# merthidayetoglu/HiCCL

Measured on AMD Instinct MI355X. Metric: GB/s device-resident N-way float bucket sum, 1 GB/input; % HBM peak, higher is better.
Workload: dtype f32

## Files before the change

### hiccl_amd/csrc/oneshot.cpp

```cpp
#include <string.h>

#include "plan.h"

using namespace hiccl_impl;

namespace {

uint32_t log2u(int v) {
  uint32_t l = 0;
  while (v > 1) {
    v >>= 1;
    l++;
  }
  return l;
}

int reduce_via_table(int dtype, const Cfg &c, void *out, const void *const *in, int n, size_t count,
                     hipStream_t s) {
  DescTable t((size_t)n, unit_pkts(c.engine, dtype, c.acc, c.unroll));
  t.add(out, in, (size_t)n, count, esize(dtype));
  const std::vector<char> host = t.image();
  char *dmem = nullptr;
  if (int e = check_hip(hipMallocAsync((void **)&dmem, host.size(), s), "hiccl_reduce: hipMallocAsync")) return e;
  if (int e = check_hip(hipMemcpyAsync(dmem, host.data(), host.size(), hipMemcpyHostToDevice, s),
                        "hiccl_reduce: table upload")) {
    (void)hipFreeAsync(dmem, s);
    return e;
  }
  PlanArgs a;
  memset(&a, 0, sizeof(a));
  t.bind(a, dmem);
  a.t_begin = 0;
  a.t_end = t.units;
  const int pol = plan_pol(c.store == kPolStoreSys ? HICCL_PEER_STORES : 0);
  if (int e = launch_plan(a, dtype, c, n, current_device(), s, pol)) {
    (void)hipFreeAsync(dmem, s);
    return e;
  }
  return check_hip(hipFreeAsync(dmem, s), "hiccl_reduce: hipFreeAsync");
}

}

extern "C" {

int hiccl_reduce_ex(int dtype, void *out, const void *const *in, int n, size_t count,
                    void *stream, const hiccl_reduce_config_t *cfg) {
  const size_t esz = esize(dtype);
  if (!esz) return fail(hipErrorInvalidValue, "hiccl_reduce: unknown dtype " + std::to_string(dtype));
  if (count == 0) return 0;
  if (dtype == HICCL_BYTES && n != 1) return fail(hipErrorInvalidValue, "hiccl_reduce: HICCL_BYTES copies need n == 1");
  if (int e = check_buffers(out, in, n, count, esz)) return e;
  if (int e = check_cfg(cfg, "hiccl_reduce")) return e;
  hipStream_t s = (hipStream_t)stream;
  const int dev = current_device();
  Split sp = split_on(out, count, esz);
  Cfg c = oneshot_cfg(dtype, cfg, sp.npkt, (uint64_t)count * esz, n, dev);
  if (n > kMaxArgInputs) {
    const std::string why = plan_shape_error(c, dtype);
    if (!why.empty()) return fail(hipErrorInvalidValue, "hiccl_reduce_ex: n > 64 inputs run on the plan kernel: " + why);
    if (capturing(s, false))
      return fail(hipErrorStreamCaptureUnsupported,
                  "hiccl_reduce: n > 64 inputs cannot be captured into a graph (use a plan)");
    return reduce_via_table(dtype, c, out, in, n, count, s);
  }

  single_fn fn = single_for(dtype, c);
  if (!fn)
    return fail(hipErrorInvalidValue, "hiccl_reduce_ex: unsupported config (block " +
                                          std::to_string(c.block) + ", unroll " +
                                          std::to_string(c.unroll) + ", nt " +
                                          std::to_string(c.nt) + ", store " +
                                          std::to_string(c.store) + ", engine " +
                                          std::to_string(c.engine) + ") for this dtype");

  SingleArgs a;
  memset(&a, 0, sizeof(a));
  a.out = (char *)out;
  a.npkt = sp.npkt;
  a.head = sp.head;
  a.tail = sp.tail;
  a.n = (uint32_t)n;
  a.ntiles = tiles_for(sp.npkt, (uint64_t)c.block * c.unroll);
  for (int k = 0; k < n; k++) a.in[k] = (const char *)in[k];

  const LaunchShape L = launch_shape(c, n, a.ntiles, device_cus(dev));
  a.grab = L.grab;
  a.drain = (uint32_t)c.drain;
  a.order = log2u(c.order);
  a.sched = L.dynamic ? ticket_counter(dev, s) : nullptr;
  fn(a, dim3((unsigned)L.grid), s);
  return check_hip(hipGetLastError(), "hiccl_reduce: launch");
}

int hiccl_reduce(int dtype, void *out, const void *const *in, int n, size_t count, void *stream) {
  return hiccl_reduce_ex(dtype, out, in, n, count, stream, nullptr);
}

int hiccl_reduce_f32(float *out, const float *const *in, int n, size_t count, void *stream) {
  return hiccl_reduce_ex(HICCL_FLOAT32, out, (const void *const *)in, n, count, stream, nullptr);
}

int hiccl_reduce_bf16(uint16_t *out, const uint16_t *const *in, int n, size_t count,
                      void *stream) {
  return hiccl_reduce_ex(HICCL_BFLOAT16, out, (const void *const *)in, n, count, stream, nullptr);
}

int hiccl_reduce_auto_choice_ex(int dtype, const hiccl_reduce_config_t *cfg, size_t count, double n, int cus,
                                int *engine, int *unroll, int *blocks_per_cu, int *dynamic, int *store_policy) {
  const size_t esz = esize(dtype);
  if (!esz) return fail(hipErrorInvalidValue, "auto_choice: unknown dtype");
  if (cus <= 0 || n < 0) return fail(hipErrorInvalidValue, "auto_choice: cus must be > 0 and n >= 0");
  if (int e = check_cfg(cfg, "auto_choice")) return e;
  CusOverride scoped(cus);
  const uint64_t npkt = (uint64_t)count * esz / kPacket;
  const Cfg c = oneshot_cfg(dtype, cfg, npkt, (uint64_t)count * esz, n, -1);
  const bool has = n > kMaxArgInputs ? plan_shape_error(c, dtype).empty() : single_for(dtype, c) != nullptr;
  if (!has) return fail(hipErrorInvalidValue, "auto_choice: no kernel for this config and dtype");
  const uint64_t units = tiles_for(npkt, (uint64_t)c.block * c.unroll);
  const LaunchShape L = launch_shape(c, n, units, cus);
  if (engine) *engine = c.engine;
  if (unroll) *unroll = c.unroll;
  if (blocks_per_cu) *blocks_per_cu = c.bpc;
  if (dynamic) *dynamic = L.dynamic ? 1 : 0;
  if (store_policy) *store_policy = c.store + 1;
  return 0;
}

int hiccl_reduce_auto_choice(int dtype, int acc, size_t count, double n, int cus, int *engine, int *unroll,
                             int *blocks_per_cu, int *dynamic) {
  hiccl_reduce_config_t z;
  memset(&z, 0, sizeof(z));
  z.acc = acc;
  return hiccl_reduce_auto_choice_ex(dtype, &z, count, n, cus, engine, unroll, blocks_per_cu, dynamic, nullptr);
}

}
```

### hiccl_amd/csrc/policy.cpp

```cpp
#include "policy.h"

namespace hiccl_impl {

namespace {

constexpr uint64_t kDynMinUnitsPerWG = 32;
constexpr double kDynMinInputs = 5;
constexpr double kTicketTiles = 9;
constexpr uint64_t kTileMinTicketsPerWG = 64;

constexpr int kWideUnroll = 8;
constexpr uint64_t kWideMinTicketsPerWG = 128;

constexpr uint64_t kWtMaxBytes = 32ull << 20;
constexpr uint64_t kWtMaxBytesReduce = 256ull << 20;
inline uint64_t wt_cap(double n) { return n >= 1.5 ? kWtMaxBytesReduce : kWtMaxBytes; }

constexpr int kDefBpc = 1;
constexpr int kSmallBpc = 4;
constexpr uint64_t kPhaseMinChunksPerCU = 1;

uint32_t default_grab(int engine, double n, int unroll = kDefUnroll) {
  if (engine == HICCL_ENGINE_PHASE || unroll >= kWideUnroll) return 1u;
  const double g = kTicketTiles / (n + 1.0);
  return g <= 1.0 ? 1u : (uint32_t)(g + 0.999);
}

int auto_wide_unroll(uint64_t npkt, double n, int dtype, const Cfg &c, int dev) {
  if (!tuned_type(dtype, c.acc) || n < 1.5 || n >= kDynMinInputs) return 0;
  if ((c.block && c.block != kDefBlock) || c.nt != kDefPol % 10 || c.store != kDefPol / 10) return 0;
  if (npkt / ((uint64_t)kDefBlock * kWideUnroll) < kWideMinTicketsPerWG * (uint64_t)device_cus(dev)) return 0;
  return n < 2.5 ? 2 * kWideUnroll : kWideUnroll;
}

int auto_engine(uint64_t npkt, double n, int dtype, const Cfg &c, int dev) {
  const int acc = c.acc;
  if (auto_wide_unroll(npkt, n, dtype, c, dev)) return HICCL_ENGINE_TILE;
  const bool packed_ok = !(dtype == HICCL_BFLOAT16 && acc == HICCL_ACC_WIDE);
  const bool wt = c.wt;
  const bool wt_f32 = wt && dtype == HICCL_FLOAT32;
  const bool wt_many = wt && tuned_type(dtype, acc);
  if (n >= kDynMinInputs && packed_ok && !wt_many) {
    const uint64_t tickets = npkt / ((uint64_t)kDefBlock * kDefUnroll) / default_grab(HICCL_ENGINE_TILE, n);
    if (tickets >= kTileMinTicketsPerWG * (uint64_t)device_cus(dev)) return HICCL_ENGINE_TILE;
  }
  const uint64_t chunk = (uint64_t)kPhBlock * phase_p(dtype, acc);
  const uint64_t cus = (uint64_t)device_cus(dev);
  const uint64_t per_cu = npkt / (cus * chunk);
  const bool big_chunk = chunk >= 8192;
  const uint64_t chunks = (npkt + chunk - 1) / chunk;
  const double round_eff = chunks ? (double)chunks / (double)(((chunks + cus - 1) / cus) * cus) : 0.0;
  if (n < 2.5) return per_cu > 16 && round_eff >= 0.89 ? HICCL_ENGINE_PHASE : HICCL_ENGINE_TILE;
  if (n >= 2.5 && n < 3.5 && wt_f32) return HICCL_ENGINE_TILE;
  if (n < kDynMinInputs) return per_cu >= 4 && round_eff >= 0.89 ? HICCL_ENGINE_PHASE : HICCL_ENGINE_TILE;
  const bool enough = per_cu >= 1 || (n >= 16 && big_chunk);
  return enough && round_eff >= (big_chunk ? 0.7 : 0.8) ? HICCL_ENGINE_PHASE : HICCL_ENGINE_TILE;
}

int auto_bpc(int engine, uint64_t npkt, int dtype, int acc, int dev) {
  const uint64_t chunk = (uint64_t)kPhBlock * phase_p(dtype, acc);
  return engine == HICCL_ENGINE_TILE && npkt < kPhaseMinChunksPerCU * (uint64_t)device_cus(dev) * chunk
             ? kSmallBpc
             : kDefBpc;
}

int auto_unroll(uint64_t npkt, int dtype, int acc, int dev) {
  return tuned_type(dtype, acc) && npkt < 2ull * device_cus(dev) * kDefBlock * kDefUnroll ? 2 : kDefUnroll;
}

}

Cfg resolve(const hiccl_reduce_config_t *c) {
  Cfg r{0, 0, 0, kDefPol % 10, HICCL_ACC_NATIVE, 0, kDefPol / 10, HICCL_ENGINE_AUTO, HICCL_SCHED_AUTO, 0, 0, true,
        false, 0};
  if (c) {
    r.block = c->block;
    r.unroll = c->unroll;
    if (c->blocks_per_cu) r.bpc = c->blocks_per_cu;
    if (c->nontemporal) r.nt = c->nontemporal - 1;
    r.acc = c->acc;
    r.grid = c->grid;
    if (c->store_policy) r.store = c->store_policy - 1;
    r.store_auto = c->store_policy == 0;
    r.engine = c->engine;
    r.schedule = c->schedule;
    r.grab = c->grab;
    r.drain = c->drain;
    r.order = c->order;
  }
  return r;
}

int check_cfg(const hiccl_reduce_config_t *c, const std::string &who) {
  if (!c) return 0;
  if (c->acc != HICCL_ACC_NATIVE && c->acc != HICCL_ACC_WIDE) return fail(hipErrorInvalidValue, who + ": bad acc mode");
  if (c->engine < HICCL_ENGINE_AUTO || c->engine > HICCL_ENGINE_PHASE)
    return fail(hipErrorInvalidValue, who + ": bad engine");
  if (c->schedule < HICCL_SCHED_AUTO || c->schedule > HICCL_SCHED_DYNAMIC)
    return fail(hipErrorInvalidValue, who + ": bad schedule");
  if (c->grab < 0 || c->grab > 4096) return fail(hipErrorInvalidValue, who + ": bad grab");
  if (c->order < 0 || c->order > 4096 || (c->order & (c->order - 1)))
    return fail(hipErrorInvalidValue, who + ": order must be 0 or a power of two <= 4096");
  if (c->blocks_per_cu < 0 || c->blocks_per_cu > 64) return fail(hipErrorInvalidValue, who + ": blocks_per_cu");
  if (c->grid < 0) return fail(hipErrorInvalidValue, who + ": grid < 0");
  return 0;
}

bool wt_by_size(const Cfg &raw, int dtype, double n, uint64_t out_bytes) {
  const bool u_ok = !raw.unroll || wt_unroll(raw.unroll) || raw.engine == HICCL_ENGINE_PHASE;
  return raw.store_auto && raw.nt == kDefPol % 10 && u_ok && out_bytes <= wt_cap(dtype == HICCL_BYTES ? 1.0 : n);
}

void finish_cfg(Cfg &c, uint64_t npkt, double n, int dtype, int dev) {
  if (c.engine == HICCL_ENGINE_AUTO)
    c.engine = (c.block || c.unroll) ? HICCL_ENGINE_TILE : auto_engine(npkt, n, dtype, c, dev);
  if (c.engine == HICCL_ENGINE_PHASE) {
    if (!c.block) c.block = kPhBlock;
    if (!c.unroll) c.unroll = phase_p(dtype, c.acc);
  } else {
    if (!c.block) c.block = kDefBlock;
    if (!c.unroll) {
      const int wide = auto_wide_unroll(npkt, n, dtype, c, dev);
      c.unroll = wide ? wide : auto_unroll(npkt, dtype, c.acc, dev);
    }
  }
  if (!c.bpc) c.bpc = auto_bpc(c.engine, npkt, dtype, c.acc, dev);
}

Cfg oneshot_cfg(int dtype, const hiccl_reduce_config_t *cfg, uint64_t npkt, uint64_t out_bytes, double n,
                int dev) {
  const Cfg raw = resolve(cfg);
  Cfg c = raw;
  c.wt = wt_by_size(raw, dtype, n, out_bytes);
  finish_cfg(c, npkt, n, dtype, dev);
  if (!c.wt) return c;
  Cfg w = c;
  w.store = kPolStoreSys;
  if (n > kMaxArgInputs ? pick_plan(dtype, w.acc, w.engine, w.unroll, plan_pol(HICCL_PEER_STORES)) != nullptr
                        : single_for(dtype, w) != nullptr)
    return w;
  c = raw;
  finish_cfg(c, npkt, n, dtype, dev);
  return c;
}

int plan_pol(int peer) {
  return 10 * ((peer & HICCL_PEER_STORES) ? kPolStoreSys : kDefPol / 10) +
         ((peer & HICCL_PEER_LOADS) ? kPolLoadSys : kDefPol % 10);
}

uint64_t unit_pkts(int engine, int dtype, int acc, int unroll) {
  return engine == HICCL_ENGINE_PHASE ? (uint64_t)kPhBlock * phase_p(dtype, acc)
                                      : (uint64_t)kDefBlock * (unroll ? unroll : kDefUnroll);
}

std::string plan_shape_error(const Cfg &c, int dtype) {
  if (c.nt != kDefPol % 10 || (c.store != kDefPol / 10 && c.store != kPolStoreSys))
    return "plan kernels load nt (nontemporal 2) and store nt (store_policy 2), system-scope write-through "
           "(store_policy 4) or either by the launch's size (store_policy 0)";
  if (c.drain) return "plan kernels do not support drain";
  if (c.order != 0 && c.order != 1) return "plan kernels run their units in linear order (order 0)";
  if (c.engine == HICCL_ENGINE_PHASE) {
    if (c.block != kPhBlock || c.unroll != phase_p(dtype, c.acc))
      return "plan kernels run the PHASE engine in its default shape only (block 512, unroll " +
             std::to_string(phase_p(dtype, c.acc)) + ")";
    return "";
  }
  if (c.block != kDefBlock) return "plan kernels run the TILE engine at block 256 only";
  const bool wt = c.store == kPolStoreSys;
  if (wt && !wt_unroll(c.unroll))
    return "write-through plan kernels (store_policy 4) run the TILE engine at unroll 4 (f32 / bf16: 2 or 4) only";
  if (!pick_plan(dtype, c.acc, HICCL_ENGINE_TILE, c.unroll, plan_pol(wt ? HICCL_PEER_STORES : 0)))
    return "plan kernels run the TILE engine at unroll 4 (f32 / bf16: 1, 2, 4, 8 or 16) only";
  return "";
}

LaunchShape launch_shape(const Cfg &c, double n, uint64_t units, int cus) {
  LaunchShape L;
  L.grid = c.grid > 0 ? (uint64_t)c.grid : (uint64_t)cus * c.bpc;
  if (L.grid > units) L.grid = units;
  L.grab = c.grab > 0 ? (uint32_t)c.grab : default_grab(c.engine, n, c.unroll);
  const bool auto_static = c.engine != HICCL_ENGINE_TILE || (n < kDynMinInputs && c.unroll < kWideUnroll);
  L.dynamic = c.schedule != HICCL_SCHED_STATIC && !(c.schedule == HICCL_SCHED_AUTO && auto_static) &&
              (units + L.grab - 1) / L.grab >= kDynMinUnitsPerWG * L.grid;
  return L;
}

}
```

### hiccl_amd/csrc/policy.h

```cpp
#pragma once

#include <string>

#include "runtime.h"

namespace hiccl_impl __attribute__((visibility("hidden"))) {

struct Cfg {
  int block, unroll, bpc, nt, acc, grid, store, engine, schedule, grab, drain;
  bool store_auto;
  bool wt;
  int order;
  int pol() const { return store * 10 + nt; }
};

Cfg resolve(const hiccl_reduce_config_t *c);

int check_cfg(const hiccl_reduce_config_t *c, const std::string &who);

bool wt_by_size(const Cfg &raw, int dtype, double n, uint64_t out_bytes);
inline bool wt_unroll(int unroll) { return unroll == 2 || unroll == kDefUnroll; }

void finish_cfg(Cfg &c, uint64_t npkt, double n, int dtype, int dev);

Cfg oneshot_cfg(int dtype, const hiccl_reduce_config_t *cfg, uint64_t npkt, uint64_t out_bytes, double n, int dev);
inline single_fn single_for(int dtype, const Cfg &c) {
  return pick_single(dtype, c.acc, c.engine, c.block, c.unroll, c.pol());
}

int plan_pol(int peer);
uint64_t unit_pkts(int engine, int dtype, int acc, int unroll);
std::string plan_shape_error(const Cfg &c, int dtype);

struct LaunchShape {
  uint64_t grid;
  uint32_t grab;
  bool dynamic;
};
LaunchShape launch_shape(const Cfg &c, double n, uint64_t units, int cus);

}
```

### hiccl_amd/csrc/reduce.hip

```cpp

#include <hip/hip_runtime.h>

#include <stdint.h>

#include <type_traits>

#include "../../include/hiccl_reduce.h"
#include "kernels.h"

using namespace hiccl_impl;

namespace {


typedef uint32_t u32x4 __attribute__((ext_vector_type(4)));
typedef uint32_t u32x4u __attribute__((ext_vector_type(4), aligned(1)));
typedef float f32x4 __attribute__((ext_vector_type(4)));
typedef double f64x2 __attribute__((ext_vector_type(2)));
typedef uint64_t u64x2 __attribute__((ext_vector_type(2)));
typedef float f32x8 __attribute__((ext_vector_type(8)));
typedef __bf16 bf16x2 __attribute__((ext_vector_type(2)));

typedef __amdgpu_buffer_rsrc_t rsrc_t;
constexpr int kRsrcFlags = 0x00020000;

__device__ __forceinline__ rsrc_t make_rsrc(const char *base, uint32_t nbytes) {
  return __builtin_amdgcn_make_buffer_rsrc((void *)base, (short)0, (int)nbytes, kRsrcFlags);
}

template <int POL>
__device__ __forceinline__ u32x4 load_pkt(rsrc_t r, uint32_t voff) {
  constexpr int lp = POL % 10;
  return __builtin_amdgcn_raw_buffer_load_b128(r, (int)voff, 0, lp == 1 ? 2 : lp == kPolLoadSys ? 17 : 0);
}

template <int POL>
__device__ __forceinline__ void store_pkt(rsrc_t r, uint32_t voff, u32x4 v) {
  constexpr int sp = POL / 10;
  __builtin_amdgcn_raw_buffer_store_b128(v, r, (int)voff, 0, sp == 1 ? 2 : sp == 2 ? 16 : sp == kPolStoreSys ? 17 : 0);
}

__device__ __forceinline__ float bf_lo(uint32_t w) { return __uint_as_float(w << 16); }
__device__ __forceinline__ float bf_hi(uint32_t w) { return __uint_as_float(w & 0xffff0000u); }
__device__ __forceinline__ uint32_t bf_pack(float lo, float hi) {
  bf16x2 v = {(__bf16)lo, (__bf16)hi};
  return __builtin_bit_cast(uint32_t, v);
}
__device__ __forceinline__ uint16_t bf_round(float f) {
  return __builtin_bit_cast(uint16_t, (__bf16)f);
}

template <class T>
__device__ __forceinline__ T gld(const char *p) {
  return *(const __attribute__((address_space(1))) T *)p;
}
template <class T>
__device__ __forceinline__ void gst(char *p, T v) {
  *(__attribute__((address_space(1))) T *)p = v;
}


struct OpF32 {
  static constexpr bool kWidens = false;
  static constexpr int kEsz = 4;
  typedef f32x4 acc_t;
  __device__ static acc_t zero() { return (f32x4)(0.0f); }
  __device__ static acc_t add(acc_t a, u32x4 p) { return a + __builtin_bit_cast(f32x4, p); }
  __device__ static u32x4 pack(acc_t a) { return __builtin_bit_cast(u32x4, a); }
  typedef float sacc_t;
  __device__ static sacc_t szero() { return 0.0f; }
  __device__ static sacc_t sadd(sacc_t a, const char *p) { return a + gld<float>(p); }
  __device__ static void sstore(char *p, sacc_t a) { gst<float>(p, a); }
};

struct OpF64 {
  static constexpr bool kWidens = false;
  static constexpr int kEsz = 8;
  typedef f64x2 acc_t;
  __device__ static acc_t zero() { return (f64x2)(0.0); }
  __device__ static acc_t add(acc_t a, u32x4 p) { return a + __builtin_bit_cast(f64x2, p); }
  __device__ static u32x4 pack(acc_t a) { return __builtin_bit_cast(u32x4, a); }
  typedef double sacc_t;
  __device__ static sacc_t szero() { return 0.0; }
  __device__ static sacc_t sadd(sacc_t a, const char *p) { return a + gld<double>(p); }
  __device__ static void sstore(char *p, sacc_t a) { gst<double>(p, a); }
};

struct OpU64 {
  static constexpr bool kWidens = false;
  static constexpr int kEsz = 8;
  typedef u64x2 acc_t;
  __device__ static acc_t zero() { return (u64x2)(0); }
  __device__ static acc_t add(acc_t a, u32x4 p) { return a + __builtin_bit_cast(u64x2, p); }
  __device__ static u32x4 pack(acc_t a) { return __builtin_bit_cast(u32x4, a); }
  typedef uint64_t sacc_t;
  __device__ static sacc_t szero() { return 0; }
  __device__ static sacc_t sadd(sacc_t a, const char *p) { return a + gld<uint64_t>(p); }
  __device__ static void sstore(char *p, sacc_t a) { gst<uint64_t>(p, a); }
};

struct OpI32 {
  static constexpr bool kWidens = false;
  static constexpr int kEsz = 4;
  typedef u32x4 acc_t;
  __device__ static acc_t zero() { return (u32x4)(0u); }
  __device__ static acc_t add(acc_t a, u32x4 p) { return a + p; }
  __device__ static u32x4 pack(acc_t a) { return a; }
  typedef uint32_t sacc_t;
  __device__ static sacc_t szero() { return 0u; }
  __device__ static sacc_t sadd(sacc_t a, const char *p) { return a + gld<uint32_t>(p); }
  __device__ static void sstore(char *p, sacc_t a) { gst<uint32_t>(p, a); }
};

__device__ __forceinline__ uint32_t bf_pack_opaque(float lo, float hi) {
  uint32_t r;
  asm("v_cvt_pk_bf16_f32 %0, %1, %2" : "=v"(r) : "v"(lo), "v"(hi));
  return r;
}

struct OpBF16 {
  static constexpr bool kWidens = true;
  static constexpr int kEsz = 2;
  typedef u32x4 acc_t;
  __device__ static acc_t zero() { return (u32x4)(0u); }
  __device__ static acc_t add(acc_t a, u32x4 p) {
    acc_t r;
#pragma unroll
    for (int w = 0; w < 4; w++)
      r[w] = bf_pack_opaque(bf_lo(a[w]) + bf_lo(p[w]), bf_hi(a[w]) + bf_hi(p[w]));
    return r;
  }
  __device__ static u32x4 pack(acc_t a) { return a; }
  typedef float sacc_t;
  __device__ static sacc_t szero() { return 0.0f; }
  __device__ static sacc_t sadd(sacc_t a, const char *p) {
    float s = a + __uint_as_float((uint32_t)(gld<uint16_t>(p)) << 16);
    return __uint_as_float((uint32_t)bf_round(s) << 16);
  }
  __device__ static void sstore(char *p, sacc_t a) { gst<uint16_t>(p, bf_round(a)); }
};

struct OpBF16Wide {
  static constexpr bool kWidens = true;
  static constexpr int kEsz = 2;
  typedef f32x8 acc_t;
  __device__ static acc_t zero() { return (f32x8)(0.0f); }
  __device__ static acc_t add(acc_t a, u32x4 p) {
#pragma unroll
    for (int w = 0; w < 4; w++) {
      a[2 * w] += bf_lo(p[w]);
      a[2 * w + 1] += bf_hi(p[w]);
    }
    return a;
  }
  __device__ static u32x4 pack(acc_t a) {
    u32x4 r;
#pragma unroll
    for (int w = 0; w < 4; w++) r[w] = bf_pack(a[2 * w], a[2 * w + 1]);
    return r;
  }
  typedef float sacc_t;
  __device__ static sacc_t szero() { return 0.0f; }
  __device__ static sacc_t sadd(sacc_t a, const char *p) {
    return a + __uint_as_float((uint32_t)(gld<uint16_t>(p)) << 16);
  }
  __device__ static void sstore(char *p, sacc_t a) { gst<uint16_t>(p, bf_round(a)); }
};

struct OpRaw {
  static constexpr bool kWidens = false;
  static constexpr int kEsz = 1;
  typedef u32x4 acc_t;
  __device__ static acc_t zero() { return (u32x4)(0u); }
  __device__ static acc_t add(acc_t, u32x4 p) { return p; }
  __device__ static u32x4 pack(acc_t a) { return a; }
  typedef uint8_t sacc_t;
  __device__ static sacc_t szero() { return 0; }
  __device__ static sacc_t sadd(sacc_t, const char *p) { return gld<uint8_t>(p); }
  __device__ static void sstore(char *p, sacc_t a) { gst<uint8_t>(p, a); }
};


struct ArgInputs {
  const char *const *p;
  __device__ const char *operator()(int k) const { return p[k]; }
};

template <class Op, int POL = 11, class Inputs>
__device__ __forceinline__ void scalar_part(char *out, Inputs in, uint32_t n, uint32_t head,
                                            uint64_t npkt, uint32_t tail, int tid) {
  constexpr int V = kPacket / Op::kEsz;
  if (tid >= (int)(head + tail)) return;
  if constexpr (POL % 10 == kPolLoadSys) __builtin_amdgcn_fence(__ATOMIC_ACQUIRE, "");
  uint64_t e = (tid < (int)head) ? (uint64_t)tid : (uint64_t)head + npkt * V + (tid - head);
  uint64_t off = e * Op::kEsz;
  typename Op::sacc_t acc = Op::szero();
  for (uint32_t k = 0; k < n; k++) acc = Op::sadd(acc, in(k) + off);
  Op::sstore(out + off, acc);
  if constexpr (POL / 10 == kPolStoreSys) __builtin_amdgcn_fence(__ATOMIC_RELEASE, "");
}

template <class Op, int U, int G, int POL, class Inputs>
__device__ __forceinline__ void group_at(typename Op::acc_t (&acc)[U], Inputs in, uint32_t g,
                                         uint64_t tile_off, uint32_t tile_bytes,
                                         const uint32_t (&voff)[U]) {
  rsrc_t r[G];
#pragma unroll
  for (int j = 0; j < G; j++) r[j] = make_rsrc(in(g + j) + tile_off, tile_bytes);
  u32x4 x[G][U];
#pragma unroll
  for (int j = 0; j < G; j++) {
#pragma unroll
    for (int u = 0; u < U; u++) x[j][u] = load_pkt<POL>(r[j], voff[u]);
    __builtin_amdgcn_sched_barrier(0);
  }
#pragma unroll
  for (int j = 0; j < G; j++) {
#pragma unroll
    for (int u = 0; u < U; u++) acc[u] = Op::add(acc[u], x[j][u]);
  }
}

struct NoHook {
  __device__ void operator()() const {}
};

template <class Op, int U, int POL, class Inputs, class Hook = NoHook>
__device__ __forceinline__ void tile_body(char *outb, Inputs in, uint32_t n, uint64_t tile_off,
                                          uint32_t tile_bytes, const uint32_t (&voff)[U],
                                          Hook before_store = Hook()) {
  typename Op::acc_t acc[U];
#pragma unroll
  for (int u = 0; u < U; u++) acc[u] = Op::zero();
  constexpr uint32_t GM = U >= 8 ? 32 / U : 8;
  uint32_t g = 0;
  for (; g + GM <= n; g += GM) group_at<Op, U, GM, POL>(acc, in, g, tile_off, tile_bytes, voff);
  switch (n - g) {
    case 1: group_at<Op, U, 1, POL>(acc, in, g, tile_off, tile_bytes, voff); break;
    case 2: if constexpr (GM > 2) group_at<Op, U, 2, POL>(acc, in, g, tile_off, tile_bytes, voff); break;
    case 3: if constexpr (GM > 3) group_at<Op, U, 3, POL>(acc, in, g, tile_off, tile_bytes, voff); break;
    case 4: if constexpr (GM > 4) group_at<Op, U, 4, POL>(acc, in, g, tile_off, tile_bytes, voff); break;
    case 5: if constexpr (GM > 5) group_at<Op, U, 5, POL>(acc, in, g, tile_off, tile_bytes, voff); break;
    case 6: if constexpr (GM > 6) group_at<Op, U, 6, POL>(acc, in, g, tile_off, tile_bytes, voff); break;
    case 7: if constexpr (GM > 7) group_at<Op, U, 7, POL>(acc, in, g, tile_off, tile_bytes, voff); break;
    default: break;
  }
  before_store();
  rsrc_t w = make_rsrc(outb + tile_off, tile_bytes);
#pragma unroll
  for (int u = 0; u < U; u++) store_pkt<POL>(w, voff[u], Op::pack(acc[u]));
}

template <class Op, int P, int POL, class Inputs, class Hook = NoHook>
__device__ __forceinline__ void chunk_body(char *outb, Inputs in, uint32_t n, uint64_t off,
                                           uint32_t nbytes, const uint32_t (&voff)[P],
                                           Hook before_store = Hook()) {
  typename Op::acc_t acc[P];
#pragma unroll
  for (int p = 0; p < P; p++) acc[p] = Op::zero();
  if (n > 0) {
    u32x4 x[P], y[P];
    {
      rsrc_t r = make_rsrc(in(0) + off, nbytes);
#pragma unroll
      for (int p = 0; p < P; p++) x[p] = load_pkt<POL>(r, voff[p]);
    }
    uint32_t j = 0;
    for (; j + 2 <= n; j += 2) {
      rsrc_t ry = make_rsrc(in(j + 1) + off, nbytes);
#pragma unroll
      for (int p = 0; p < P; p++) y[p] = load_pkt<POL>(ry, voff[p]);
      __builtin_amdgcn_sched_barrier(0);
#pragma unroll
      for (int p = 0; p < P; p++) {
        acc[p] = Op::add(acc[p], x[p]);
        if constexpr (Op::kWidens) __builtin_amdgcn_sched_barrier(0);
      }
      __builtin_amdgcn_sched_barrier(0);
      const bool more = j + 2 < n;
      rsrc_t rx = make_rsrc(in(more ? j + 2 : j + 1) + off, more ? nbytes : 0u);
#pragma unroll
      for (int p = 0; p < P; p++) x[p] = load_pkt<POL>(rx, voff[p]);
      __builtin_amdgcn_sched_barrier(0);
#pragma unroll
      for (int p = 0; p < P; p++) {
        acc[p] = Op::add(acc[p], y[p]);
        if constexpr (Op::kWidens) __builtin_amdgcn_sched_barrier(0);
      }
      __builtin_amdgcn_sched_barrier(0);
    }
    if (n & 1) {
#pragma unroll
      for (int p = 0; p < P; p++) acc[p] = Op::add(acc[p], x[p]);
    }
  }
  before_store();
  rsrc_t w = make_rsrc(outb + off, nbytes);
#pragma unroll
  for (int p = 0; p < P; p++) store_pkt<POL>(w, voff[p], Op::pack(acc[p]));
}

constexpr int kTile = 0;
constexpr int kPhase = 1;

template <class Op, int U, int POL, int ENG, class Inputs, class Hook>
__device__ __forceinline__ void unit_body(char *outb, Inputs in, uint32_t n, uint64_t off,
                                          uint32_t nbytes, const uint32_t (&voff)[U], Hook hook) {
  if constexpr (ENG == kPhase)
    chunk_body<Op, U, POL>(outb, in, n, off, nbytes, voff, hook);
  else
    tile_body<Op, U, POL>(outb, in, n, off, nbytes, voff, hook);
}

template <class Inner>
struct Shifted {
  Inner in;
  uint64_t shift;
  __device__ const char *operator()(int k) const { return in(k) + shift; }
};

__device__ __forceinline__ void drain_stores(uint32_t drain) {
  if (drain) asm volatile("s_waitcnt vmcnt(0)" ::: "memory");
}

template <class Body>
__device__ __forceinline__ void for_each_unit(uint32_t *sched, uint32_t grab, uint64_t t0, uint64_t t1,
                                              Body body, uint32_t drain = 0) {
  if (!sched) {
    for (uint64_t t = t0 + blockIdx.x; t < t1; t += gridDim.x) {
      body(t, [] {});
      drain_stores(drain);
    }
    return;
  }
  __shared__ uint32_t s_next[2];
  if (threadIdx.x == 0)
    s_next[0] = __hip_atomic_fetch_add(&sched[0], 1u, __ATOMIC_RELAXED, __HIP_MEMORY_SCOPE_AGENT);
  __syncthreads();
  uint64_t t = t0 + (uint64_t)s_next[0] * grab;
  int slot = 1;
  while (t < t1) {
    uint32_t nxt;
    if (threadIdx.x == 0)
      nxt = __hip_atomic_fetch_add(&sched[0], 1u, __ATOMIC_RELAXED, __HIP_MEMORY_SCOPE_AGENT);
    const uint64_t tend = (t + grab < t1) ? t + grab : t1;
    for (uint64_t u = t; u < tend; u++) {
      const bool last = u + 1 == tend;
      body(u, [&]() {
        if (last && threadIdx.x == 0) s_next[slot] = nxt;
      });
      drain_stores(drain);
    }
    __syncthreads();
    t = t0 + (uint64_t)s_next[slot] * grab;
    slot ^= 1;
  }
  if (threadIdx.x == 0) {
    const uint32_t prev = __hip_atomic_fetch_add(&sched[1], 1u, __ATOMIC_ACQ_REL, __HIP_MEMORY_SCOPE_AGENT);
    if (prev == gridDim.x - 1) {
      __hip_atomic_store(&sched[0], 0u, __ATOMIC_RELAXED, __HIP_MEMORY_SCOPE_AGENT);
      __hip_atomic_store(&sched[1], 0u, __ATOMIC_RELAXED, __HIP_MEMORY_SCOPE_AGENT);
    }
  }
}

__device__ __forceinline__ uint64_t tile_order(uint64_t t, uint64_t n, uint32_t L) {
  if (!L) return t;
  const uint64_t S = 1ull << L, q = n >> L, r = n & (S - 1);
  uint64_t seg, idx;
  if (t < (q << L)) {
    seg = t & (S - 1);
    idx = t >> L;
  } else {
    seg = t - (q << L);
    idx = q;
  }
  return seg * q + (seg < r ? seg : r) + idx;
}


template <class Op, int BLOCK, int U, int POL, int ENG>
__global__ __launch_bounds__(BLOCK) void k_reduce_single(SingleArgs a) {
  const int tid = threadIdx.x;
  uint32_t voff[U];
#pragma unroll
  for (int u = 0; u < U; u++) voff[u] = (uint32_t)((u * BLOCK + tid) * kPacket);
  ArgInputs raw{a.in};
  if (blockIdx.x == 0) scalar_part<Op>(a.out, raw, a.n, a.head, a.npkt, a.tail, tid);
  if (a.npkt == 0) return;
  const uint64_t shift = (uint64_t)a.head * Op::kEsz;
  Shifted<ArgInputs> in{raw, shift};
  char *outb = a.out + shift;
  constexpr uint64_t TILE = (uint64_t)BLOCK * U;
  for_each_unit(a.sched, a.grab, 0, a.ntiles, [&](uint64_t u, auto hook) {
    const uint64_t t = tile_order(u, a.ntiles, a.order);
    const uint64_t pkt0 = t * TILE;
    const uint64_t left = a.npkt - pkt0;
    const uint32_t tile_bytes = (uint32_t)((left < TILE ? left : TILE) * kPacket);
    unit_body<Op, U, POL, ENG>(outb, in, a.n, pkt0 * kPacket, tile_bytes, voff, hook);
  }, a.drain);
}

typedef const char *const __attribute__((address_space(4))) ConstPtr;

struct TableInputs {
  const char *const *p;
  __device__ const char *operator()(int k) const { return ((ConstPtr *)p)[k]; }
};

typedef const PlanDesc __attribute__((address_space(4))) ConstDesc;
typedef const uint32_t __attribute__((address_space(4))) ConstU32;

__device__ __forceinline__ PlanDesc load_desc(const PlanDesc *desc, uint32_t c) {
  const ConstDesc *q = (const ConstDesc *)desc + c;
  PlanDesc d;
  d.out = q->out;
  d.npkt = q->npkt;
  d.tile_begin = q->tile_begin;
  d.n = q->n;
  d.head = q->head;
  d.tail = q->tail;
  d.pad = 0;
  return d;
}

template <class Op, int BLOCK, int U, int POL, int ENG>
__global__ __launch_bounds__(BLOCK) void k_reduce_plan(PlanArgs a) {
  const int tid = threadIdx.x;
  uint32_t voff[U];
#pragma unroll
  for (int u = 0; u < U; u++) voff[u] = (uint32_t)((u * BLOCK + tid) * kPacket);
  constexpr uint64_t TILE = (uint64_t)BLOCK * U;
  for_each_unit(a.sched, a.grab, a.t_begin, a.t_end, [&](uint64_t t, auto hook) {
    const uint32_t c = a.unit_comp ? ((ConstU32 *)a.unit_comp)[t] : 0u;
    const PlanDesc d = load_desc(a.desc, c);
    const uint64_t lt = t - d.tile_begin;
    TableInputs raw{a.ptrs + (uint64_t)c * a.stride};
    if (lt == 0) scalar_part<Op, POL>(d.out, raw, d.n, d.head, d.npkt, d.tail, tid);
    const uint64_t pkt0 = lt * TILE;
    if (pkt0 >= d.npkt) {
      hook();
      return;
    }
    const uint64_t shift = (uint64_t)d.head * Op::kEsz;
    Shifted<TableInputs> in{raw, shift};
    const uint64_t left = d.npkt - pkt0;
    const uint32_t tile_bytes = (uint32_t)((left < TILE ? left : TILE) * kPacket);
    unit_body<Op, U, POL, ENG>(d.out + shift, in, d.n, pkt0 * kPacket, tile_bytes, voff, hook);
  });
}


__device__ __forceinline__ uint64_t splitmix64(uint64_t z) {
  z += 0x9e3779b97f4a7c15ull;
  z = (z ^ (z >> 30)) * 0xbf58476d1ce4e5b9ull;
  z = (z ^ (z >> 27)) * 0x94d049bb133111ebull;
  return z ^ (z >> 31);
}

__device__ __forceinline__ float uniform_f32(uint64_t key, uint64_t i) {
  uint64_t h = splitmix64(key + i);
  return (float)(uint32_t)(h >> 40) * (1.0f / 8388608.0f) - 1.0f;
}

template <int DT>
__global__ __launch_bounds__(256) void k_fill(char *out, uint64_t count, uint64_t key,
                                              uint64_t first) {
  for (uint64_t i = (uint64_t)blockIdx.x * 256 + threadIdx.x; i < count;
       i += (uint64_t)gridDim.x * 256) {
    float v = uniform_f32(key, first + i);
    if constexpr (DT == HICCL_FLOAT32) ((float *)out)[i] = v;
    if constexpr (DT == HICCL_FLOAT64) ((double *)out)[i] = (double)v;
    if constexpr (DT == HICCL_BFLOAT16) ((uint16_t *)out)[i] = bf_round(v);
  }
}

__global__ __launch_bounds__(256) void k_copy(u32x4 *__restrict__ dst,
                                              const u32x4 *__restrict__ src, uint64_t npkt) {
  constexpr int U = 4;
  const uint64_t stride = (uint64_t)gridDim.x * 256 * U;
  for (uint64_t b = (uint64_t)blockIdx.x * 256 * U; b < npkt; b += stride) {
    u32x4 v[U];
#pragma unroll
    for (int u = 0; u < U; u++) {
      uint64_t p = b + u * 256 + threadIdx.x;
      if (p < npkt) v[u] = src[p];
    }
#pragma unroll
    for (int u = 0; u < U; u++) {
      uint64_t p = b + u * 256 + threadIdx.x;
      if (p < npkt) dst[p] = v[u];
    }
  }
}

__global__ void k_copy_bytes(char *dst, const char *src, uint64_t nbytes) {
  for (uint64_t i = threadIdx.x; i < nbytes; i += blockDim.x) dst[i] = src[i];
}


__global__ __launch_bounds__(64) void k_sigwait_phases(SigPhaseArgs a) {
  const uint32_t lane = threadIdx.x;
  const uint32_t add = a.epoch_dev ? __hip_atomic_load(a.epoch_dev, __ATOMIC_RELAXED, __HIP_MEMORY_SCOPE_AGENT) : 0u;
  uint32_t s0 = 0, w0 = 0;
  for (uint32_t p = 0; p < a.nphase; p++) {
    const uint32_t epoch = a.epoch[p] + add;
    const uint32_t s1 = a.sig_end[p], w1 = a.wait_end[p];
    if (s0 + lane < s1) {
      if (a.light)
        __hip_atomic_store(a.sig[s0 + lane], epoch, __ATOMIC_RELAXED, __HIP_MEMORY_SCOPE_SYSTEM);
      else
        __hip_atomic_store(a.sig[s0 + lane], epoch, __ATOMIC_RELEASE, __HIP_MEMORY_SCOPE_SYSTEM);
    }
    if (w0 + lane < w1) {
      const uint32_t *f = a.wait[w0 + lane];
      const uint64_t t0 = __builtin_amdgcn_s_memrealtime();
      auto poll = [&]() { return __hip_atomic_load(f, __ATOMIC_RELAXED, __HIP_MEMORY_SCOPE_SYSTEM); };
      while ((int32_t)(poll() - epoch) < 0) {
        __builtin_amdgcn_s_sleep(2);
        if (a.err && __hip_atomic_load(a.err, __ATOMIC_RELAXED, __HIP_MEMORY_SCOPE_SYSTEM)) break;
        if (__builtin_amdgcn_s_memrealtime() - t0 > a.timeout_ticks) {
          if (a.err) __hip_atomic_store(a.err, 1u, __ATOMIC_RELAXED, __HIP_MEMORY_SCOPE_SYSTEM);
          break;
        }
      }
    }
    if (!a.light) __atomic_thread_fence(__ATOMIC_ACQUIRE);
    __syncthreads();
    s0 = s1;
    w0 = w1;
  }
}

__global__ __launch_bounds__(64) void k_counter_add(uint32_t *ctr, uint32_t v) {
  if (threadIdx.x == 0) __hip_atomic_fetch_add(ctr, v, __ATOMIC_RELAXED, __HIP_MEMORY_SCOPE_AGENT);
}


constexpr int kProgPol = kDefPol;

__device__ __forceinline__ void prog_phases(const ProgArgs &a, uint32_t count, uint32_t lane, uint32_t add) {
  for (uint32_t p = 0; p < count; p++) {
    const ConstU32 *q = (const ConstU32 *)&a.phase[p];
    const uint32_t s0 = q[0], s1 = q[1], w0 = q[2], w1 = q[3];
    const uint32_t epoch = a.epoch[p] + add;
    for (uint32_t i = s0 + lane; i < s1; i += 64) {
      uint32_t *f = ((uint32_t *const __attribute__((address_space(4))) *)a.sig)[i];
      if (a.light)
        __hip_atomic_store(f, epoch, __ATOMIC_RELAXED, __HIP_MEMORY_SCOPE_SYSTEM);
      else
        __hip_atomic_store(f, epoch, __ATOMIC_RELEASE, __HIP_MEMORY_SCOPE_SYSTEM);
    }
    for (uint32_t i = w0 + lane; i < w1; i += 64) {
      const uint32_t *f = ((const uint32_t *const __attribute__((address_space(4))) *)a.wait)[i];
      const uint64_t t0 = __builtin_amdgcn_s_memrealtime();
      while ((int32_t)(__hip_atomic_load(f, __ATOMIC_RELAXED, __HIP_MEMORY_SCOPE_SYSTEM) - epoch) < 0) {
        __builtin_amdgcn_s_sleep(2);
        if (a.err && __hip_atomic_load(a.err, __ATOMIC_RELAXED, __HIP_MEMORY_SCOPE_SYSTEM)) break;
        if (__builtin_amdgcn_s_memrealtime() - t0 > a.timeout_ticks) {
          if (a.err) __hip_atomic_store(a.err, 1u, __ATOMIC_RELAXED, __HIP_MEMORY_SCOPE_SYSTEM);
          break;
        }
      }
    }
    if (!a.light) __builtin_amdgcn_fence(__ATOMIC_ACQUIRE, "");
    __builtin_amdgcn_fence(__ATOMIC_RELEASE, "wavefront");
    __builtin_amdgcn_wave_barrier();
    __builtin_amdgcn_fence(__ATOMIC_ACQUIRE, "wavefront");
  }
}

__device__ __forceinline__ void prog_gate_wait(const ProgArgs &a, uint64_t seq) {
  const uint64_t t0 = __builtin_amdgcn_s_memrealtime();
  uint32_t nap = 1;
  while (__hip_atomic_load(a.gate, __ATOMIC_RELAXED, __HIP_MEMORY_SCOPE_AGENT) != seq) {
    for (uint32_t i = 0; i < nap; i++) __builtin_amdgcn_s_sleep(2);
    if (nap < 8) nap <<= 1;
    if (a.err && __hip_atomic_load(a.err, __ATOMIC_RELAXED, __HIP_MEMORY_SCOPE_SYSTEM)) return;
    if (__builtin_amdgcn_s_memrealtime() - t0 > a.timeout_ticks) {
      if (a.err) __hip_atomic_store(a.err, 2u, __ATOMIC_RELAXED, __HIP_MEMORY_SCOPE_SYSTEM);
      return;
    }
  }
}

template <class Op, int U, int POL>
__device__ __forceinline__ void prog_unit_of(const PlanDesc &d, TableInputs raw, uint64_t lt, int tid,
                                             const uint32_t (&voff)[U]) {
  constexpr uint64_t TILE = (uint64_t)kProgBlock * U;
  if (lt == 0) scalar_part<Op, POL>(d.out, raw, d.n, d.head, d.npkt, d.tail, tid);
  const uint64_t pkt0 = lt * TILE;
  if (pkt0 >= d.npkt) return;
  const uint64_t shift = (uint64_t)d.head * Op::kEsz;
  Shifted<TableInputs> in{raw, shift};
  const uint64_t left = d.npkt - pkt0;
  const uint32_t tile_bytes = (uint32_t)((left < TILE ? left : TILE) * kPacket);
  tile_body<Op, U, POL>(d.out + shift, in, d.n, pkt0 * kPacket, tile_bytes, voff);
}

template <class Op, int U>
__device__ __forceinline__ void prog_unit_peer(uint32_t peer, const PlanDesc &d, TableInputs raw, uint64_t lt,
                                               int tid, const uint32_t (&voff)[U]) {
  constexpr int L = kProgPol % 10, S = kProgPol / 10;
  switch (peer & 3u) {
    case 0: prog_unit_of<Op, U, kProgPol>(d, raw, lt, tid, voff); break;
    case 1: prog_unit_of<Op, U, 10 * kPolStoreSys + L>(d, raw, lt, tid, voff); break;
    case 2: prog_unit_of<Op, U, 10 * S + kPolLoadSys>(d, raw, lt, tid, voff); break;
    default: prog_unit_of<Op, U, 10 * kPolStoreSys + kPolLoadSys>(d, raw, lt, tid, voff); break;
  }
}

template <class Op, int U>
__global__ __launch_bounds__(kProgBlock) void k_program(ProgArgs a) {
  const int tid = threadIdx.x;
  uint32_t voff[U];
#pragma unroll
  for (int u = 0; u < U; u++) voff[u] = (uint32_t)((u * kProgBlock + tid) * kPacket);
  if (a.nphase) {
    const uint32_t add = a.epoch_dev ? __hip_atomic_load(a.epoch_dev, __ATOMIC_RELAXED, __HIP_MEMORY_SCOPE_AGENT) : 0u;
    const uint64_t seq = a.seq + add;
    if (blockIdx.x == 0) {
      if (tid < 64) {
        prog_phases(a, a.nphase, (uint32_t)tid, add);
        if (tid == 0) {
          if (a.light)
            __hip_atomic_store(a.gate, seq, __ATOMIC_RELAXED, __HIP_MEMORY_SCOPE_AGENT);
          else
            __hip_atomic_store(a.gate, seq, __ATOMIC_RELEASE, __HIP_MEMORY_SCOPE_AGENT);
        }
      }
    } else if (tid == 0) {
      prog_gate_wait(a, seq);
      if (!a.light) __builtin_amdgcn_fence(__ATOMIC_ACQUIRE, "agent");
    }
    __syncthreads();
  }
  for (uint64_t t = blockIdx.x; t < a.nunits; t += gridDim.x) {
    const uint32_t c = a.unit_comp ? ((ConstU32 *)a.unit_comp)[t] : 0u;
    const ConstDesc *q = (const ConstDesc *)a.desc + c;
    const PlanDesc d = load_desc(a.desc, c);
    const uint32_t flags = q->pad;
    TableInputs raw{a.ptrs + (uint64_t)c * a.stride};
    if (flags & 1u)
      prog_unit_peer<OpRaw, U>(flags >> 1, d, raw, t - d.tile_begin, tid, voff);
    else
      prog_unit_peer<Op, U>(flags >> 1, d, raw, t - d.tile_begin, tid, voff);
  }
}


template <int DT, class O, bool TUNED>
struct Elem {
  static constexpr int dtype = DT;
  typedef O Op;
  static constexpr bool tuned = TUNED;
};

template <class R, class F>
R with_elem(int dtype, int acc, R unknown, F f) {
  switch (dtype) {
    case HICCL_FLOAT32: return f(Elem<HICCL_FLOAT32, OpF32, true>());
    case HICCL_BFLOAT16:
      return acc == HICCL_ACC_WIDE ? f(Elem<HICCL_BFLOAT16, OpBF16Wide, false>())
                                   : f(Elem<HICCL_BFLOAT16, OpBF16, true>());
    case HICCL_FLOAT64: return f(Elem<HICCL_FLOAT64, OpF64, false>());
    case HICCL_UINT64: return f(Elem<HICCL_UINT64, OpU64, false>());
    case HICCL_INT32: return f(Elem<HICCL_INT32, OpI32, false>());
    case HICCL_BYTES: return f(Elem<HICCL_BYTES, OpRaw, false>());
    default: return unknown;
  }
}

template <class Op>
constexpr int phase_p_of() {
  return (sizeof(typename Op::acc_t) > 16 || std::is_same<Op, OpI32>::value) ? 8 : 16;
}


template <class Op, int B, int U, int POL, int ENG = kTile>
void launch_single_t(SingleArgs a, dim3 grid, hipStream_t s) {
  hipLaunchKernelGGL((k_reduce_single<Op, B, U, POL, ENG>), grid, dim3(B), 0, s, a);
}

template <class Op, int B, int U>
single_fn pick_nt(int pol) {
  switch (pol) {
    case 0: return launch_single_t<Op, B, U, 0>;
    case 1: return launch_single_t<Op, B, U, 1>;
    case 10: return launch_single_t<Op, B, U, 10>;
    case 11: return launch_single_t<Op, B, U, 11>;
    case 20: return launch_single_t<Op, B, U, 20>;
    case 21: return launch_single_t<Op, B, U, 21>;
    case 10 * kPolStoreSys + 1: return launch_single_t<Op, B, U, 10 * kPolStoreSys + 1>;
    default: return nullptr;
  }
}

template <class Op, int B>
single_fn pick_u(int u, int pol) {
  switch (u) {
    case 1: return pick_nt<Op, B, 1>(pol);
    case 2: return pick_nt<Op, B, 2>(pol);
    case 4: return pick_nt<Op, B, 4>(pol);
    case 8: return pol == kDefPol && B == 256 ? launch_single_t<Op, B, 8, kDefPol> : nullptr;
    case 16: return pol == kDefPol && B == 256 ? launch_single_t<Op, B, 16, kDefPol> : nullptr;
    default: return nullptr;
  }
}

template <class Op, bool TUNED>
single_fn pick_phase(int block, int unroll, int pol) {
  constexpr int PD = phase_p_of<Op>();
  if (block == kPhBlock && unroll == PD) {
    switch (pol) {
      case 11: return launch_single_t<Op, kPhBlock, PD, 11, kPhase>;
      case 10 * kPolStoreSys + 1: return launch_single_t<Op, kPhBlock, PD, 10 * kPolStoreSys + 1, kPhase>;
      case 1: if constexpr (TUNED) return launch_single_t<Op, kPhBlock, PD, 1, kPhase>; break;
      case 10: if constexpr (TUNED) return launch_single_t<Op, kPhBlock, PD, 10, kPhase>; break;
      case 21: if constexpr (TUNED) return launch_single_t<Op, kPhBlock, PD, 21, kPhase>; break;
      case 0: if constexpr (TUNED) return launch_single_t<Op, kPhBlock, PD, 0, kPhase>; break;
      default: break;
    }
    return nullptr;
  }
  if constexpr (TUNED) {
    if (pol != kDefPol) return nullptr;
    if (block == 1024 && unroll == 4) return launch_single_t<Op, 1024, 4, 11, kPhase>;
    if constexpr (PD == 16) {
      if (block == 512 && unroll == 8) return launch_single_t<Op, 512, 8, 11, kPhase>;
      if (block == 1024 && unroll == 8) return launch_single_t<Op, 1024, 8, 11, kPhase>;
      if (block == 256 && unroll == 16) return launch_single_t<Op, 256, 16, 11, kPhase>;
    } else {
      if (block == 512 && unroll == 4) return launch_single_t<Op, 512, 4, 11, kPhase>;
    }
  }
  return nullptr;
}

template <class Op, bool TUNED>
single_fn pick_single_op(int engine, int block, int unroll, int pol) {
  if (engine == HICCL_ENGINE_PHASE) return pick_phase<Op, TUNED>(block, unroll, pol);
  if constexpr (TUNED) {
    if (block == 256) return pick_u<Op, 256>(unroll, pol);
    if (block == 512) return pick_u<Op, 512>(unroll, pol);
    return nullptr;
  } else {
    if (block != kDefBlock || unroll != kDefUnroll) return nullptr;
    if (pol == 10 * kPolStoreSys + 1) return launch_single_t<Op, kDefBlock, kDefUnroll, 10 * kPolStoreSys + 1>;
    return pol == kDefPol ? launch_single_t<Op, kDefBlock, kDefUnroll, kDefPol> : nullptr;
  }
}


template <class Op, int ENG, int U, int POL = kDefPol>
void launch_plan_t(const PlanArgs &a, dim3 grid, hipStream_t s) {
  constexpr int B = ENG == kPhase ? kPhBlock : kDefBlock;
  hipLaunchKernelGGL((k_reduce_plan<Op, B, U, POL, ENG>), grid, dim3(B), 0, s, a);
}

template <class Op, bool TUNED, int POL>
plan_fn pick_plan_pol(int engine, int unroll) {
  constexpr bool DEF = POL == kDefPol;
  if (engine == HICCL_ENGINE_PHASE) return launch_plan_t<Op, kPhase, phase_p_of<Op>(), POL>;
  switch (unroll) {
    case 0:
    case 4: return launch_plan_t<Op, kTile, 4, POL>;
    case 2: if constexpr (TUNED) return launch_plan_t<Op, kTile, 2, POL>; break;
    case 8: if constexpr (TUNED && DEF) return launch_plan_t<Op, kTile, 8>; break;
    case 16: if constexpr (TUNED && DEF) return launch_plan_t<Op, kTile, 16>; break;
    case 1: if constexpr (TUNED && DEF) return launch_plan_t<Op, kTile, 1>; break;
    default: break;
  }
  return nullptr;
}

template <class Op, bool TUNED>
plan_fn pick_plan_eng(int engine, int unroll, int pol) {
  constexpr int L = kDefPol % 10, S = kDefPol / 10;
  switch (pol) {
    case kDefPol: return pick_plan_pol<Op, TUNED, kDefPol>(engine, unroll);
    case 10 * kPolStoreSys + L: return pick_plan_pol<Op, TUNED, 10 * kPolStoreSys + L>(engine, unroll);
    case 10 * S + kPolLoadSys: return pick_plan_pol<Op, TUNED, 10 * S + kPolLoadSys>(engine, unroll);
    case 10 * kPolStoreSys + kPolLoadSys:
      return pick_plan_pol<Op, TUNED, 10 * kPolStoreSys + kPolLoadSys>(engine, unroll);
    default: return nullptr;
  }
}


template <class Op, int U>
void launch_prog_t(const ProgArgs &a, dim3 grid, hipStream_t s) {
  hipLaunchKernelGGL((k_program<Op, U>), grid, dim3(kProgBlock), 0, s, a);
}

}


namespace hiccl_impl {

size_t esize(int dtype) {
  return with_elem(dtype, HICCL_ACC_NATIVE, (size_t)0, [](auto e) { return (size_t)decltype(e)::Op::kEsz; });
}

bool tuned_type(int dtype, int acc) {
  return with_elem(dtype, acc, false, [](auto e) { return decltype(e)::tuned; });
}

int phase_p(int dtype, int acc) {
  return with_elem(dtype, acc, 16, [](auto e) { return phase_p_of<typename decltype(e)::Op>(); });
}

single_fn pick_single(int dtype, int acc, int engine, int block, int unroll, int pol) {
  return with_elem(dtype, acc, (single_fn) nullptr, [&](auto e) {
    typedef decltype(e) E;
    return pick_single_op<typename E::Op, E::tuned>(engine, block, unroll, pol);
  });
}

plan_fn pick_plan(int dtype, int acc, int engine, int unroll, int pol) {
  return with_elem(dtype, acc, (plan_fn) nullptr, [&](auto e) {
    typedef decltype(e) E;
    return pick_plan_eng<typename E::Op, E::tuned>(engine, unroll, pol);
  });
}

prog_fn pick_prog(int dtype, int unroll) {
  return with_elem(dtype, HICCL_ACC_NATIVE, (prog_fn) nullptr, [&](auto e) -> prog_fn {
    typedef decltype(e) E;
    if constexpr (std::is_same<typename E::Op, OpBF16Wide>::value) return nullptr;
    else if (unroll != 2) return launch_prog_t<typename E::Op, 4>;
    else if constexpr (E::tuned) return launch_prog_t<typename E::Op, 2>;
    else return nullptr;
  });
}

void launch_sigwait_phases(const SigPhaseArgs &a, hipStream_t s) {
  hipLaunchKernelGGL(k_sigwait_phases, dim3(1), dim3(64), 0, s, a);
}

void launch_counter_add(uint32_t *ctr, uint32_t v, hipStream_t s) {
  hipLaunchKernelGGL(k_counter_add, dim3(1), dim3(64), 0, s, ctr, v);
}

bool launch_fill(int dtype, unsigned blocks, hipStream_t s, char *out, uint64_t count, uint64_t key, uint64_t first) {
  return with_elem(dtype, HICCL_ACC_NATIVE, false, [&](auto e) {
    typedef decltype(e) E;
    if constexpr (std::is_floating_point<typename E::Op::sacc_t>::value) {
      hipLaunchKernelGGL(k_fill<E::dtype>, dim3(blocks), dim3(256), 0, s, out, count, key, first);
      return true;
    } else {
      return false;
    }
  });
}

void launch_copy(unsigned blocks, hipStream_t s, void *dst, const void *src, uint64_t npkt) {
  hipLaunchKernelGGL(k_copy, dim3(blocks), dim3(256), 0, s, (u32x4 *)dst, (const u32x4 *)src, npkt);
}

void launch_copy_bytes(hipStream_t s, char *dst, const char *src, uint64_t nbytes) {
  hipLaunchKernelGGL(k_copy_bytes, dim3(1), dim3(64), 0, s, dst, src, nbytes);
}

}
```

Measured before the change: 6696.

## Pace dynamic tile loads with s_sleep and shrink grid for ticketed launches

For dynamically scheduled tile launches, the grid is cut to 7/8 of the default, and a short s_sleep is inserted between input loads inside each group. The aim is to ease HBM and fabric contention from too many outstanding requests. It also forces tile offsets and sizes to wavefront-uniform values via readfirstlane, and hoists creation of the output resource descriptor ahead of the accumulate loop. The risk is that fewer workgroups plus idle sleeps leave bandwidth unused if memory was not actually oversubscribed.

```diff
diff --git a/hiccl_amd/csrc/oneshot.cpp b/hiccl_amd/csrc/oneshot.cpp
--- a/hiccl_amd/csrc/oneshot.cpp
+++ b/hiccl_amd/csrc/oneshot.cpp
@@ -84,11 +84,12 @@
   a.ntiles = tiles_for(sp.npkt, (uint64_t)c.block * c.unroll);
   for (int k = 0; k < n; k++) a.in[k] = (const char *)in[k];
 
-  const LaunchShape L = launch_shape(c, n, a.ntiles, device_cus(dev));
+  LaunchShape L = launch_shape(c, n, a.ntiles, device_cus(dev), true);
+  a.sched = L.dynamic ? ticket_counter(dev, s) : nullptr;
+  if (L.dynamic && !a.sched) L = launch_shape(c, n, a.ntiles, device_cus(dev));
   a.grab = L.grab;
   a.drain = (uint32_t)c.drain;
   a.order = log2u(c.order);
-  a.sched = L.dynamic ? ticket_counter(dev, s) : nullptr;
   fn(a, dim3((unsigned)L.grid), s);
   return check_hip(hipGetLastError(), "hiccl_reduce: launch");
 }
@@ -118,7 +119,7 @@
   const bool has = n > kMaxArgInputs ? plan_shape_error(c, dtype).empty() : single_for(dtype, c) != nullptr;
   if (!has) return fail(hipErrorInvalidValue, "auto_choice: no kernel for this config and dtype");
   const uint64_t units = tiles_for(npkt, (uint64_t)c.block * c.unroll);
-  const LaunchShape L = launch_shape(c, n, units, cus);
+  const LaunchShape L = launch_shape(c, n, units, cus, n <= kMaxArgInputs);
   if (engine) *engine = c.engine;
   if (unroll) *unroll = c.unroll;
   if (blocks_per_cu) *blocks_per_cu = c.bpc;
diff --git a/hiccl_amd/csrc/policy.cpp b/hiccl_amd/csrc/policy.cpp
--- a/hiccl_amd/csrc/policy.cpp
+++ b/hiccl_amd/csrc/policy.cpp
@@ -15,6 +15,8 @@
 constexpr uint64_t kWtMaxBytes = 32ull << 20;
 constexpr uint64_t kWtMaxBytesReduce = 256ull << 20;
 inline uint64_t wt_cap(double n) { return n >= 1.5 ? kWtMaxBytesReduce : kWtMaxBytes; }
+
+constexpr uint64_t kPacedGridNum = 7, kPacedGridDen = 8;
 
 constexpr int kDefBpc = 1;
 constexpr int kSmallBpc = 4;
@@ -175,7 +177,7 @@
   return "";
 }
 
-LaunchShape launch_shape(const Cfg &c, double n, uint64_t units, int cus) {
+LaunchShape launch_shape(const Cfg &c, double n, uint64_t units, int cus, bool paced) {
   LaunchShape L;
   L.grid = c.grid > 0 ? (uint64_t)c.grid : (uint64_t)cus * c.bpc;
   if (L.grid > units) L.grid = units;
@@ -183,6 +185,8 @@
   const bool auto_static = c.engine != HICCL_ENGINE_TILE || (n < kDynMinInputs && c.unroll < kWideUnroll);
   L.dynamic = c.schedule != HICCL_SCHED_STATIC && !(c.schedule == HICCL_SCHED_AUTO && auto_static) &&
               (units + L.grab - 1) / L.grab >= kDynMinUnitsPerWG * L.grid;
+  if (paced && L.dynamic && c.engine == HICCL_ENGINE_TILE && c.grid <= 0 && L.grid >= 8)
+    L.grid = L.grid * kPacedGridNum / kPacedGridDen;
   return L;
 }
 
diff --git a/hiccl_amd/csrc/policy.h b/hiccl_amd/csrc/policy.h
--- a/hiccl_amd/csrc/policy.h
+++ b/hiccl_amd/csrc/policy.h
@@ -37,6 +37,6 @@
   uint32_t grab;
   bool dynamic;
 };
-LaunchShape launch_shape(const Cfg &c, double n, uint64_t units, int cus);
+LaunchShape launch_shape(const Cfg &c, double n, uint64_t units, int cus, bool paced = false);
 
 }
diff --git a/hiccl_amd/csrc/reduce.hip b/hiccl_amd/csrc/reduce.hip
--- a/hiccl_amd/csrc/reduce.hip
+++ b/hiccl_amd/csrc/reduce.hip
@@ -200,7 +200,9 @@
   if constexpr (POL / 10 == kPolStoreSys) __builtin_amdgcn_fence(__ATOMIC_RELEASE, "");
 }
 
-template <class Op, int U, int G, int POL, class Inputs>
+constexpr int kPaceSleep = 4;
+
+template <class Op, int U, int G, int POL, bool PACED, class Inputs>
 __device__ __forceinline__ void group_at(typename Op::acc_t (&acc)[U], Inputs in, uint32_t g,
                                          uint64_t tile_off, uint32_t tile_bytes,
                                          const uint32_t (&voff)[U]) {
@@ -213,6 +215,12 @@
 #pragma unroll
     for (int u = 0; u < U; u++) x[j][u] = load_pkt<POL>(r[j], voff[u]);
     __builtin_amdgcn_sched_barrier(0);
+    if constexpr (PACED) {
+      if (j + 1 < G) {
+        __builtin_amdgcn_s_sleep(kPaceSleep);
+        __builtin_amdgcn_sched_barrier(0);
+      }
+    }
   }
 #pragma unroll
   for (int j = 0; j < G; j++) {
@@ -222,31 +230,32 @@
 }
 
 struct NoHook {
+  static constexpr bool kDynamic = false;
   __device__ void operator()() const {}
 };
 
-template <class Op, int U, int POL, class Inputs, class Hook = NoHook>
+template <class Op, int U, int POL, bool PACED = false, class Inputs, class Hook = NoHook>
 __device__ __forceinline__ void tile_body(char *outb, Inputs in, uint32_t n, uint64_t tile_off,
                                           uint32_t tile_bytes, const uint32_t (&voff)[U],
                                           Hook before_store = Hook()) {
   typename Op::acc_t acc[U];
 #pragma unroll
   for (int u = 0; u < U; u++) acc[u] = Op::zero();
+  const rsrc_t w = make_rsrc(outb + tile_off, tile_bytes);
   constexpr uint32_t GM = U >= 8 ? 32 / U : 8;
   uint32_t g = 0;
-  for (; g + GM <= n; g += GM) group_at<Op, U, GM, POL>(acc, in, g, tile_off, tile_bytes, voff);
+  for (; g + GM <= n; g += GM) group_at<Op, U, GM, POL, PACED>(acc, in, g, tile_off, tile_bytes, voff);
   switch (n - g) {
-    case 1: group_at<Op, U, 1, POL>(acc, in, g, tile_off, tile_bytes, voff); break;
-    case 2: if constexpr (GM > 2) group_at<Op, U, 2, POL>(acc, in, g, tile_off, tile_bytes, voff); break;
-    case 3: if constexpr (GM > 3) group_at<Op, U, 3, POL>(acc, in, g, tile_off, tile_bytes, voff); break;
-    case 4: if constexpr (GM > 4) group_at<Op, U, 4, POL>(acc, in, g, tile_off, tile_bytes, voff); break;
-    case 5: if constexpr (GM > 5) group_at<Op, U, 5, POL>(acc, in, g, tile_off, tile_bytes, voff); break;
-    case 6: if constexpr (GM > 6) group_at<Op, U, 6, POL>(acc, in, g, tile_off, tile_bytes, voff); break;
-    case 7: if constexpr (GM > 7) group_at<Op, U, 7, POL>(acc, in, g, tile_off, tile_bytes, voff); break;
+    case 1: group_at<Op, U, 1, POL, PACED>(acc, in, g, tile_off, tile_bytes, voff); break;
+    case 2: if constexpr (GM > 2) group_at<Op, U, 2, POL, PACED>(acc, in, g, tile_off, tile_bytes, voff); break;
+    case 3: if constexpr (GM > 3) group_at<Op, U, 3, POL, PACED>(acc, in, g, tile_off, tile_bytes, voff); break;
+    case 4: if constexpr (GM > 4) group_at<Op, U, 4, POL, PACED>(acc, in, g, tile_off, tile_bytes, voff); break;
+    case 5: if constexpr (GM > 5) group_at<Op, U, 5, POL, PACED>(acc, in, g, tile_off, tile_bytes, voff); break;
+    case 6: if constexpr (GM > 6) group_at<Op, U, 6, POL, PACED>(acc, in, g, tile_off, tile_bytes, voff); break;
+    case 7: if constexpr (GM > 7) group_at<Op, U, 7, POL, PACED>(acc, in, g, tile_off, tile_bytes, voff); break;
     default: break;
   }
   before_store();
-  rsrc_t w = make_rsrc(outb + tile_off, tile_bytes);
 #pragma unroll
   for (int u = 0; u < U; u++) store_pkt<POL>(w, voff[u], Op::pack(acc[u]));
 }
@@ -303,13 +312,20 @@
 constexpr int kTile = 0;
 constexpr int kPhase = 1;
 
-template <class Op, int U, int POL, int ENG, class Inputs, class Hook>
+__device__ __forceinline__ uint32_t uniform32(uint32_t v) { return __builtin_amdgcn_readfirstlane(v); }
+__device__ __forceinline__ uint64_t uniform64(uint64_t v) {
+  return (uint64_t)uniform32((uint32_t)(v >> 32)) << 32 | uniform32((uint32_t)v);
+}
+
+template <class Op, int U, int POL, int ENG, bool PACED = false, class Inputs, class Hook = NoHook>
 __device__ __forceinline__ void unit_body(char *outb, Inputs in, uint32_t n, uint64_t off,
-                                          uint32_t nbytes, const uint32_t (&voff)[U], Hook hook) {
+                                          uint32_t nbytes, const uint32_t (&voff)[U], Hook hook = Hook()) {
+  const uint64_t uoff = uniform64(off);
+  const uint32_t ubytes = uniform32(nbytes);
   if constexpr (ENG == kPhase)
-    chunk_body<Op, U, POL>(outb, in, n, off, nbytes, voff, hook);
+    chunk_body<Op, U, POL>(outb, in, n, uoff, ubytes, voff, hook);
   else
-    tile_body<Op, U, POL>(outb, in, n, off, nbytes, voff, hook);
+    tile_body<Op, U, POL, PACED>(outb, in, n, uoff, ubytes, voff, hook);
 }
 
 template <class Inner>
@@ -323,12 +339,19 @@
   if (drain) asm volatile("s_waitcnt vmcnt(0)" ::: "memory");
 }
 
+template <class F>
+struct TicketHook {
+  static constexpr bool kDynamic = true;
+  F f;
+  __device__ void operator()() const { f(); }
+};
+
 template <class Body>
 __device__ __forceinline__ void for_each_unit(uint32_t *sched, uint32_t grab, uint64_t t0, uint64_t t1,
                                               Body body, uint32_t drain = 0) {
   if (!sched) {
     for (uint64_t t = t0 + blockIdx.x; t < t1; t += gridDim.x) {
-      body(t, [] {});
+      body(t, NoHook());
       drain_stores(drain);
     }
     return;
@@ -346,9 +369,10 @@
     const uint64_t tend = (t + grab < t1) ? t + grab : t1;
     for (uint64_t u = t; u < tend; u++) {
       const bool last = u + 1 == tend;
-      body(u, [&]() {
+      auto publish = [&]() {
         if (last && threadIdx.x == 0) s_next[slot] = nxt;
-      });
+      };
+      body(u, TicketHook<decltype(publish)>{publish});
       drain_stores(drain);
     }
     __syncthreads();
@@ -397,7 +421,7 @@
     const uint64_t pkt0 = t * TILE;
     const uint64_t left = a.npkt - pkt0;
     const uint32_t tile_bytes = (uint32_t)((left < TILE ? left : TILE) * kPacket);
-    unit_body<Op, U, POL, ENG>(outb, in, a.n, pkt0 * kPacket, tile_bytes, voff, hook);
+    unit_body<Op, U, POL, ENG, decltype(hook)::kDynamic>(outb, in, a.n, pkt0 * kPacket, tile_bytes, voff, hook);
   }, a.drain);
 }
 
@@ -595,7 +619,7 @@
   Shifted<TableInputs> in{raw, shift};
   const uint64_t left = d.npkt - pkt0;
   const uint32_t tile_bytes = (uint32_t)((left < TILE ? left : TILE) * kPacket);
-  tile_body<Op, U, POL>(d.out + shift, in, d.n, pkt0 * kPacket, tile_bytes, voff);
+  unit_body<Op, U, POL, kTile>(d.out + shift, in, d.n, pkt0 * kPacket, tile_bytes, voff);
 }
 
 template <class Op, int U>
```

Result: faster. 6876 (median of 6 runs) (+2.7%).
